# robustrobotics/flame_ros

Hardware: AMD Instinct MI355X
Metric: primal-dual iterations/sec on a 50000-vertex / 149966-edge Delaunay graph (higher is better)
Workload: dtype f32; 1 GPU; synthetic 50k-vertex Delaunay graph, 500 PD iterations per frame, one frame per GPU; V=50000, E=149966, parallelism=replicas1, num_tiles=256, tile_depth=4, tile_threads=1024, hipgraph=True, resident_solves_repeated=0

## Files before the change

flame_ros_amd/csrc/flame_hip.cpp:

```cpp
#include "../../include/flame_hip.h"

#include <hip/hip_runtime.h>
#include <roctracer/roctx.h>

#include <atomic>
#include <chrono>
#include <climits>
#include <cmath>
#include <cstdio>
#include <cstdlib>
#include <cstring>
#include <new>
#include <string>
#include <unordered_map>
#include <mutex>
#include <vector>

#include "delaunay_dev.h"
#include "kernels.h"
#include "plan.h"
#include "plan_dev.h"
#include "sync.h"

using namespace flamehip;
// ... 210 lines not shown
  PlanOptions opt;
  int num_cus = 0;
  int use_graph = 1;
  Plan plan;
  SyncOut sync;
  bool synced = false;
  int path = 0;

  hipStream_t stream = nullptr;
  hipStream_t stream_in = nullptr;
  DelaunayScratch dt;
  hipEvent_t ev0 = nullptr, ev1 = nullptr, ev_in = nullptr;
  hipEvent_t ev_state = nullptr;
  bool state_pending = false;
  float state_scale = 1.0f;
  bool timed = false;
  int last_launches = 0;

  float4* A[2] = {nullptr, nullptr};
  float4* B[2] = {nullptr, nullptr};
  float4* q[2] = {nullptr, nullptr};
  int cur = 0;
  int2* eij = nullptr;
  float4* ew = nullptr;
  int32_t* grow = nullptr;
  int32_t* ginc = nullptr;
  float2* pos = nullptr;
  TileDesc* tiles = nullptr;
  int32_t* t_vmap = nullptr;
  int32_t* t_emap = nullptr;
  uint2* t_eij = nullptr;
  float4* t_ew = nullptr;
  uint32_t* t_srow = nullptr;
  int32_t* tris = nullptr;
  int32_t* trow = nullptr;
  int32_t* tinc = nullptr;
  float4* tri_normals = nullptr;
  float4* vtx_normals = nullptr;
  uint8_t* tri_valid = nullptr;
  int64_t map_pixels = 0;
  uint32_t* map_owner = nullptr;
  float* map_idm = nullptr;
  float* map_dm = nullptr;
  float* map_cloud = nullptr;
  uint32_t* map_cov = nullptr;
  char* fr_dev = nullptr;
  uint32_t* dbg_key = nullptr;
  uint8_t* dbg_bgr = nullptr;
  float* dbg_feat = nullptr;
  uint64_t state_serial = 1, raster_serial = 0;
  int raster_filtered = -1;
  flame_hip_tri_params raster_tp;
  float raster_kinv[9];
  float* filter_tmp = nullptr;
  float4* mesh_pts = nullptr;
  int32_t* v_i2o_dev = nullptr;
  int32_t* v_o2i_dev = nullptr;
  int32_t* e_i2o_dev = nullptr;
  int32_t* e_o2i_dev = nullptr;
  float* dl_v = nullptr;
  float* dl_q = nullptr;
  float* dl_n = nullptr;
  int plan_device = 1;
  int plan_reuse = 1;
  int plan_mini = 1;
  bool plan_mini_used = false;
// ... 53 lines not shown
  int2* in_edges = nullptr;
  float* in_alpha = nullptr;
  float* in_beta = nullptr;
  float* in_z = nullptr;
  float* in_wgt = nullptr;
  float* in_x0 = nullptr;
  int32_t* in_tris = nullptr;
  float* in_mu = nullptr;
  float* in_var = nullptr;
  float* in_pred = nullptr;
  bool sync_on_device = false;
  bool beta_is_alpha = false;
  int32_t* dflags = nullptr;
  bool host_perms = true;
  double* partials = nullptr;
  uint8_t* cost_mask = nullptr;
  int32_t n_send_v = 0, n_send_e = 0, n_recv_v = 0, n_recv_e = 0;
  int32_t* halo_send_v = nullptr;
  int32_t* halo_send_e = nullptr;
  int32_t* halo_recv_v = nullptr;
  int32_t* halo_recv_e = nullptr;
  int profile = 0;
  unsigned long long* prof = nullptr;

  std::vector<GraphExecEntry> execs;
  CapMap caps;
  int solves_since_upload = 0;
  PinnedArena pin;
  PinnedArena pin_in;
  char* in_stage = nullptr;
  PinnedArena pout;
  char* harena = nullptr;
  bool lanes_applied = false;
  bool poll_valid = false;
  bool poll_sorted = false;

  void drop_execs() {
    for (auto& e : execs) (void)hipGraphExecDestroy(e.exec);
    execs.clear();
  }

  void free_device() {
    if (device < 0) return;
    (void)hipSetDevice(device);
    drop_execs();
    for (auto& kv : caps) {
      void** pp = reinterpret_cast<void**>(kv.first);
      if (*pp) (void)hipFree(*pp);
      *pp = nullptr;
    }
    caps.clear();
    for (int b = 0; b < 2; ++b) {
      float4** pp[3] = {&xp.hA[b], &xp.hB[b], &xp.hq[b]};
      for (int k = 0; k < 3; ++k) {
        if (*pp[k]) uncached_pool().give(device, *pp[k], xp_cap[3 * b + k]);
        *pp[k] = nullptr; xp_cap[3 * b + k] = 0;
      }
    }
    xp.prof = nullptr;
    xp.poll_v = nullptr; xp.poll_e = nullptr; xp.poll_ne = nullptr;
    xp.need_v = nullptr; xp.need_e = nullptr; xp.need_valid = false;
    pin.release();
    pin_in.release();
    pout.release();
    map_pixels = 0;
    n_send_v = n_send_e = n_recv_v = n_recv_e = 0;
// ... 178 lines not shown
  } else if (k == "host_threads") {
    if (value < 0) return FLAME_HIP_ERR_ARG;
    g->opt.host_threads = value;
  } else if (k == "tile_single_max") {
    if (value < 0 || value > 2048) return FLAME_HIP_ERR_ARG;
    g->opt.single_max = value;
  } else if (k == "debug_sub_cap") {
    g->opt.debug_sub_cap = value;
  } else if (k == "d_sign") {
    if (value != 1 && value != -1) return FLAME_HIP_ERR_ARG;
    g->opt.d_sign = value;
  } else if (k == "plan_device") {
    g->plan_device = value != 0;
  } else if (k == "plan_reuse") {
    g->plan_reuse = value != 0;
  } else if (k == "plan_mini") {
    g->plan_mini = value != 0;
  } else if (k == "stream_depth") {
    if (value < 0 || value > kMaxDepth) return FLAME_HIP_ERR_ARG;
    g->stream_depth = value;
  } else if (k == "persist") {
    g->persist = value != 0;
  } else if (k == "persist_prof") {
    if (value < 0) return FLAME_HIP_ERR_ARG;
    g->persist_prof_want = value;
  } else if (k == "one_xcd") {
    g->one_xcd_opt = value != 0;
  } else if (k == "poll_delay") {
    if (value < -1 || value > 255) return FLAME_HIP_ERR_ARG;
    g->poll_delay_opt = value;
  } else if (k == "persist_timeout_us") {
    if (value < 0) return FLAME_HIP_ERR_ARG;
    g->persist_timeout_opt = value;
  } else if (k == "need_marks") {
    g->need_marks = value != 0;
  } else if (k == "plan_timing") {
    if (value < 0 || value > 5) return FLAME_HIP_ERR_ARG;
    g->opt.timing = value;
  } else if (k == "profile") {
    g->profile = value != 0;
  } else if (k == "lds_bytes") {
    if (value < 1024) return FLAME_HIP_ERR_ARG;
    g->opt.lds_bytes = value;
  } else {
    return FLAME_HIP_ERR_ARG;
  }
  return 0;
}

int flame_hip_get_info(const flame_hip_graph* g, const char* key, int64_t* value) {
  if (!g || !key || !value) return FLAME_HIP_ERR_ARG;
  const std::string k(key);
  const Plan& P = g->plan;
  if (k == "V") *value = g->V;
  else if (k == "E") *value = g->E;
  else if (k == "T") *value = g->T;
  else if (k == "path") *value = g->path;
  else if (k == "num_tiles") *value = (int64_t)P.tiles.size();
  else if (k == "tile_threads") *value = P.tile_threads;
  else if (k == "tile_ept") *value = P.tile_ept;
  else if (k == "tile_vpt") *value = P.tile_vpt;
  else if (k == "tile_depth") *value = P.tile_depth;
  else if (k == "tile_lds_bytes") *value = P.tile_lds_bytes;
  else if (k == "tile_slot12") *value = P.tile_slot12 ? 1 : 0;
  else if (k == "tile_fat") *value = P.tile_fat ? 1 : 0;
  else if (k == "stall_hook_build") *value = tile_stall_hook_build() ? 1 : 0;
// ... 347 lines not shown

int flame_hip_graph_upload(flame_hip_graph* g, const float* pos, const int32_t* edges,
                           const float* alpha, const float* beta, const float* z,
                           const float* wgt, const float* x0, const int32_t* tris) {
  RoctxRange roctx_("flame_hip_graph_upload");
  if (!g) return FLAME_HIP_ERR_ARG;
  const int32_t V = g->V, E = g->E;
  if (edges != g->sync.edges.data()) g->synced = false;
  g->sync_on_device = false;
  g->beta_is_alpha = false;
  if ((V > 0 && (!pos || !z || !wgt)) || (E > 0 && (!edges || !alpha || !beta)))
    return FLAME_HIP_ERR_ARG;
  g->uploaded = false;
  const GraphOptScope opt_scope(g, V);
  int rc;
  auto device_plan = [&]() -> int {
    int r = upload_device_plan(g, pos, edges, alpha, beta, z, wgt, x0, tris);
    if (r <= 0) {
      (void)hipStreamSynchronize(g->stream);
      (void)hipStreamSynchronize(g->stream_in);
    }
    return r;
  };
  if (g->device >= 0) {
    HIPCHK(hipSetDevice(g->device));
    HIPCHK(wait_last_solve(g));
    HIPCHK(hipStreamSynchronize(g->stream));
    persist_discard(g);
    HIPCHK(hipStreamSynchronize(g->stream_in));
    HIPCHK(g->planner.wait_maps());
    g->drop_execs();
    g->solves_since_upload = 0;
    g->lanes_applied = false;
    rc = device_plan();
    if (rc < 0) return rc;
  } else {
    rc = 0;
  }
  bool dev_plan = rc == 1;
  if (!dev_plan) {
    if (!all_finite(pos, 2 * (size_t)V) || !all_finite(z, V) || !all_finite(wgt, V) ||
        !all_finite(alpha, E) || !all_finite(beta, E) || (x0 && !all_finite(x0, V)))
      return FLAME_HIP_ERR_NAN;
    g->plan.on_device = false;
    g->host_perms = true;
    const bool auto_single = g->device >= 0 && g->plan_device && g->opt.tile_own <= 0 && g->opt.batch_voff.empty() &&
                             plan_sizing(g->opt, V, E).single;
    g->opt.single_only = auto_single;
    rc = build_plan(g->opt, V, E, g->T, pos, edges, alpha, beta, tris, &g->plan);
    g->opt.single_only = false;
    if (rc == kPlanSingleNoFit) {
      g->single_cap = std::min(g->single_cap, std::max(V - 1, 0));
      g->opt.single_max = std::min(g->opt.single_max, g->single_cap);
      rc = device_plan();
      if (rc < 0) return rc;
      dev_plan = rc == 1;
      if (!dev_plan) {
        g->plan.on_device = false;
        g->host_perms = true;
        rc = build_plan(g->opt, V, E, g->T, pos, edges, alpha, beta, tris, &g->plan);
      }
    }
    if (!dev_plan && rc != 0) return rc;
  }
  const Plan& P = g->plan;
  if (!dev_plan) {
// ... 185 lines not shown
        if (!(sc > 0.0f)) sc = 1.0f;
      }
      auto al = [](size_t v) { return (v + 63) & ~(size_t)63; };
      const size_t o_tris = 0, o_pos = al(sizeof(int32_t) * 3 * (size_t)T), o_mu = o_pos + al(sizeof(float2) * (size_t)V);
      const size_t o_var = o_mu + al(sizeof(float) * (size_t)V), o_pred = o_var + al(sizeof(float) * (size_t)V);
      const size_t in_total = o_pred + (prediction ? al(sizeof(float) * (size_t)V) : 0);
      if ((rc = dev_alloc(g->caps, &g->in_stage, in_total))) return rc;
      HIPCHK(g->pin_in.reserve(in_total));
      if (!tris_dev) std::memcpy(g->pin_in.base + o_tris, tris, sizeof(int32_t) * 3 * (size_t)T);
      std::memcpy(g->pin_in.base + o_pos, pos, sizeof(float2) * (size_t)V);
      std::memcpy(g->pin_in.base + o_mu, idepth_mu, sizeof(float) * (size_t)V);
      std::memcpy(g->pin_in.base + o_var, idepth_var, sizeof(float) * (size_t)V);
      if (prediction) std::memcpy(g->pin_in.base + o_pred, prediction, sizeof(float) * (size_t)V);
      const char* src = g->pin_in.base;
      lap("H2D all");
      DevPlanner::MiniSync ms;
      ms.tris = tris_dev ? tris_dev : reinterpret_cast<const int32_t*>(src + o_tris);
      ms.pos = reinterpret_cast<const float2*>(src + o_pos);
      ms.mu = reinterpret_cast<const float*>(src + o_mu);
      ms.var = reinterpret_cast<const float*>(src + o_var);
      ms.pred = (use_pred) ? reinterpret_cast<const float*>(src + o_pred) : nullptr;
      ms.scale = sc;
      ms.adaptive = sp->adaptive_data_weights; ms.init_pred = sp->init_with_prediction;
      ms.z = g->in_z; ms.wgt = g->in_wgt; ms.x0 = g->in_x0; ms.edges = g->in_edges; ms.alpha = g->in_alpha;
      ms.dflags = g->dflags;
      g->planner.offer_mini(ms);
      const int32_t V0 = g->V, E0 = g->E, T0 = g->T;
      g->V = V; g->E = expected_E; g->T = T;
      g->uploaded = false;
      g->n_send_v = g->n_send_e = g->n_recv_v = g->n_recv_e = 0;
      g->drop_execs();
      g->solves_since_upload = 0;
      g->lanes_applied = false;
      g->beta_is_alpha = true;
      g->spec_edges = true;
      rc = upload_device_plan(g, nullptr, nullptr, nullptr, nullptr, nullptr, nullptr, nullptr, nullptr, true, true);
      g->spec_edges = false;
      g->planner.withdraw_mini();
      if (g->planner.mini_used() && rc == 1) {
        g->plan_mini_used = true;
        g->euler_backoff = 0;
        g->euler_off = (int32_t)((int64_t)g->E - V - T);
        if ((rc = finish_upload(g))) return rc;
        g->synced = true;
        g->sync_on_device = true;
        g->sync.scale = sc;
        if (scale) *scale = sc;
        return 0;
      }
      if (rc < 0) return rc;
      (void)hipStreamSynchronize(s);
      if (rc == 2 && g->planner.mini_used()) {
        g->euler_backoff = std::min(16, std::max(1, 2 * g->euler_backoff));
        g->euler_skip = g->euler_backoff;
        expected_E = -1;
      }
      g->V = V0; g->E = E0; g->T = T0;
      HIPCHK(hipMemsetAsync(g->dflags, 0, 8 * sizeof(int32_t), s));
    }
    if (tris_dev) {
      HIPCHK(hipMemcpyAsync(g->in_tris, tris_dev, sizeof(int32_t) * 3 * (size_t)T, hipMemcpyDeviceToDevice, s));
    } else {
      HIPCHK(stage(g->in_tris, tris, sizeof(int32_t) * 3 * (size_t)T));
      HIPCHK(staged_for());
    }
    lap("H2D triangles");
    HIPCHK(g->planner.edges_from_tris(s, V, T, g->in_tris, g->in_pos, g->in_edges, g->in_alpha, &E, &index_error, g->dflags,
                                      [&]() {
                                        stage_err = stage(g->in_mu, idepth_mu, sizeof(float) * (size_t)V);
                                        if (stage_err == hipSuccess) stage_err = stage(g->in_var, idepth_var, sizeof(float) * (size_t)V);
                                        if (stage_err == hipSuccess && prediction)
                                          stage_err = stage(g->in_pred, prediction, sizeof(float) * (size_t)V);
                                        if (stage_err == hipSuccess) stage_err = staged_for();
                                        vrc = validate();
                                        if (vrc == 0 && sp->rescale_data) {
                                          double acc = 0.0;
                                          for (int32_t v = 0; v < V; ++v) acc += (double)idepth_mu[v];
                                          sc = (float)(acc / (double)V);
                                          if (!(sc > 0.0f)) sc = 1.0f;
                                        }
                                      }, expected_E,
                                      [&]() {
                                        hipError_t e = stage(g->in_pos, pos, sizeof(float2) * (size_t)V);
                                        return e != hipSuccess ? e : staged_for();
                                      }));
    HIPCHK(stage_err);
    lap("edges_from_tris");
    if (vrc || index_error) g->uploaded = false;
    if (vrc) return vrc;
    if (index_error) return FLAME_HIP_ERR_ARG;
    HIPCHK(g->planner.sync_data(s, V, g->in_mu, g->in_var, use_pred ? g->in_pred : nullptr, sc, sp->adaptive_data_weights,
                                sp->init_with_prediction, g->in_z, g->in_wgt, g->in_x0, g->dflags));
    g->V = V; g->E = E; g->T = T;
    g->uploaded = false;
    g->n_send_v = g->n_send_e = g->n_recv_v = g->n_recv_e = 0;
    g->drop_execs();
    g->solves_since_upload = 0;
    g->lanes_applied = false;
    g->beta_is_alpha = true;
    g->spec_edges = expected_E >= 0;
    rc = upload_device_plan(g, nullptr, nullptr, nullptr, nullptr, nullptr, nullptr, nullptr, nullptr, true, true);
    g->spec_edges = false;
    if (rc == 2) {
      E = g->true_edges;
      g->euler_backoff = std::min(16, std::max(1, 2 * g->euler_backoff));
      g->euler_skip = g->euler_backoff;
      if (E < 0 || E > 3 * (int64_t)T) return FLAME_HIP_ERR_ARG;
      g->E = E;
      rc = upload_device_plan(g, nullptr, nullptr, nullptr, nullptr, nullptr, nullptr, nullptr, nullptr, true, true);
    } else if (expected_E >= 0) {
      g->euler_backoff = 0;
    }
    if (rc == 1 || rc == 0) g->euler_off = (int32_t)((int64_t)g->E - V - T);
    if (rc <= 0) (void)hipStreamSynchronize(s);
    if (rc < 0) return rc;
    if (rc == 1) {
      if ((rc = finish_upload(g))) return rc;
      g->synced = true;
      g->sync_on_device = true;
      g->sync.scale = sc;
      if (scale) *scale = sc;
      return 0;
    }
  }
  if ((rc = validate())) return rc;
  if (tris_dev && !(tris = g->dt.host_list())) return FLAME_HIP_ERR_HIP;
  rc = graph_sync_host(*sp, V, T, pos, idepth_mu, idepth_var, tris, prediction, &g->sync);
  if (rc) return rc;
  const int32_t E = (int32_t)(g->sync.edges.size() / 2);
  if ((rc = flame_hip_graph_resize(g, V, E, T))) return rc;
  const SyncOut& S = g->sync;
// ... 248 lines not shown
    return 1;
  }
  g->queued.clear(); g->qsnap_valid = false;
  const bool can = g->persist_used && unchecked <= 1 && g->state_serial == g->solve_serial + (uint64_t)own_marks && g->last_iters > 0;
  g->persist_used = false;
  if (!can) {
    g->uploaded = false;
    return FLAME_HIP_ERR_STATE;
  }
  hipStream_t s = g->last_stream ? g->last_stream : g->stream;
  int cur_out = 0, launches = 0;
  HIPCHK(hipEventRecord(g->ev0, s));
  g->persist_skip_once = true;
  int rc = enqueue_iterations(g, g->last_sp, g->last_iters, s, g->last_src, &cur_out, &launches);
  g->persist_skip_once = false;
  if (rc) return rc;
  g->cur = cur_out;
  g->state_serial++;
  g->last_launches = launches;
  HIPCHK(hipEventRecord(g->ev1, s));
  ++g->persist_recovered;
  return 1;
}

static int enqueue_iterations(flame_hip_graph* g, const SolveParams& sp, int32_t num_iters,
                              hipStream_t s, int cur, int* cur_out, int* launches) {
  const Plan& P = g->plan;
  *launches = 0;
  g->persist_used = false;
  if (g->path == FLAME_HIP_PATH_TILE) {
    TileArgs a;
    a.tiles = g->tiles; a.t_vmap = g->t_vmap; a.t_emap = g->t_emap; a.t_eij = g->t_eij;
    a.t_ew = g->t_ew; a.t_srow = g->t_srow; a.p = sp; a.ntiles = (int32_t)P.tiles.size();
    a.prof = g->prof;
    a.slot12 = P.tile_slot12 ? 1 : 0;
    a.fat = P.tile_fat ? 1 : 0;
    if (persist_applies(g, num_iters) && persist_lease_take(g, s, P.tile_fat && P.tile_depth <= 2)) {
      PersistBufs& x = g->xp;
      int rc;
      if (!g->persist_err) {
        HIPCHK(hipHostMalloc(reinterpret_cast<void**>(&g->persist_err), 64, hipHostMallocDefault));
        *g->persist_err = 0;
      }
      if (!x.prof || g->persist_prof_set != g->persist_prof_want) {
        if ((rc = dev_alloc(g->caps, &x.prof, 16))) return rc;
        int32_t w[16] = {0, 0, 0, 0, 0, 0, 0, 0, 0, 0, 0, 0, 0, 0, 0, 0};
        int want = g->persist_prof_want;
        if (want > 0) { w[0] = 1; w[1] = want - 1; }
        HIPCHK(memcpy_sync(s, x.prof, w, sizeof(w), hipMemcpyHostToDevice));
        g->persist_prof_set = g->persist_prof_want;
      }
      const int rounds = (num_iters + P.tile_depth - 1) / P.tile_depth;
      bool rezero = g->persist_base > (1 << 23);
      if (rezero) g->persist_base = 0;
      const bool want_sorted = g->solves_since_upload > 0;
      if (!g->poll_valid || (want_sorted && !g->poll_sorted)) {
        size_t nv_loc = 0, ne_loc = 0;
        for (const TileDesc& D : P.tiles) { nv_loc += (size_t)D.n_ext; ne_loc += (size_t)D.e_loc; }
        if ((rc = dev_alloc(g->caps, &x.poll_v, nv_loc + 1)) || (rc = dev_alloc(g->caps, &x.poll_e, ne_loc + 1)) ||
            (rc = dev_alloc(g->caps, &x.poll_ne, P.tiles.size())))
          return rc;
        x.need_valid = false;
        if (want_sorted && g->need_marks && P.tile_fat) {
          if ((rc = dev_alloc(g->caps, &x.need_v, std::max<size_t>((size_t)g->V, 1))) || (rc = dev_alloc(g->caps, &x.need_e, std::max<size_t>((size_t)g->E, 1))))
            return rc;
          HIPCHK(hipMemsetAsync(x.need_v, 0, sizeof(int32_t) * std::max<size_t>((size_t)g->V, 1), s));
          HIPCHK(hipMemsetAsync(x.need_e, 0, sizeof(int32_t) * std::max<size_t>((size_t)g->E, 1), s));
          x.need_valid = true;
        }
        HIPCHK(launch_poll_lists(s, (int32_t)P.tiles.size(), g->tiles, g->t_vmap, g->t_emap, g->t_eij, x.poll_v, x.poll_e, x.poll_ne, want_sorted,
                                 x.need_valid ? x.need_v : nullptr, x.need_valid ? x.need_e : nullptr));
        g->poll_sorted = want_sorted;
        x.stage_bytes = 0;
        for (const TileDesc& D : P.tiles) x.stage_bytes = std::max(x.stage_bytes, persist_stage_bytes(D));
        g->poll_valid = true;
      }
      for (int b = 0; b < 2; ++b) {
        float4** pp[3] = {&x.hA[b], &x.hB[b], &x.hq[b]};
        const size_t nn[3] = {(size_t)g->V, (size_t)g->V, (size_t)std::max(g->E, 1)};
        for (int k = 0; k < 3; ++k) {
          bool fresh = false;
          if ((rc = dev_alloc_uncached(g->device, pp[k], &g->xp_cap[3 * b + k], nn[k], &fresh))) return rc;
          if (fresh || rezero) HIPCHK(hipMemsetAsync(*pp[k], 0, g->xp_cap[3 * b + k], s));
        }
      }
      PersistBufs xl = x;
      g->one_xcd_used = false;
      if (g->one_xcd_opt && P.tiles.size() <= (size_t)kOneXcdTiles && g->num_cus >= 256 && one_xcd_allowed(g->device)) {
        for (int b = 0; b < 2; ++b) {
          float4** pp[3] = {&g->cA[b], &g->cB[b], &g->cq[b]};
          const size_t nn[3] = {(size_t)g->V, (size_t)g->V, (size_t)std::max(g->E, 1)};
          for (int k = 0; k < 3; ++k) {
            if ((rc = dev_alloc(g->caps, pp[k], nn[k]))) return rc;
            const size_t cap_now = g->caps[(void*)pp[k]];
            if (g->c_zeroed[3 * b + k] != (void*)*pp[k] || g->c_zeroed_cap[3 * b + k] != cap_now || rezero) {
              HIPCHK(hipMemsetAsync(*pp[k], 0, cap_now, s));
              g->c_zeroed[3 * b + k] = (void*)*pp[k];
              g->c_zeroed_cap[3 * b + k] = cap_now;
            }
          }
          xl.hA[b] = g->cA[b]; xl.hB[b] = g->cB[b]; xl.hq[b] = g->cq[b];
        }
        xl.one_xcd = 1;
// ... 44 lines not shown
      HIPCHK(launch_primal(s, g->V, g->grow, g->ginc, g->ew, g->q[cur], g->A[cur], g->B[cur], sp));
      *launches += 2;
    }
  }
  *cur_out = cur;
  return 0;
}

int flame_hip_solve(flame_hip_graph* g, const flame_hip_params* p, int32_t num_iters,
                    void* stream) {
  RoctxRange roctx_("flame_hip_solve");
  int rc = require_device(g);
  if (rc) return rc;
  if (!p || num_iters < 0) return FLAME_HIP_ERR_ARG;
  if (!std::isfinite(p->data_factor) || !std::isfinite(p->step_x) || !std::isfinite(p->step_q) ||
      !std::isfinite(p->theta) || std::isnan(p->x_min) || std::isnan(p->x_max))
    return FLAME_HIP_ERR_NAN;
  HIPCHK(hipSetDevice(g->device));
  hipStream_t s = stream ? (hipStream_t)stream : g->stream;
  SolveParams sp;
  sp.lambda = p->data_factor; sp.tau = p->step_x; sp.sigma = p->step_q; sp.theta = p->theta;
  sp.x_min = p->x_min; sp.x_max = p->x_max;
  sp.tl = p->step_x * p->data_factor;
  HIPCHK(order_after_state(g, s));
  if (g->path == FLAME_HIP_PATH_TILE && g->opt.lane_order == 1 && !g->lanes_applied &&
      g->solves_since_upload > 0 && num_iters > 0 && g->V > 0) {
    int e_max = 0;
    for (const TileDesc& D : g->plan.tiles) e_max = std::max(e_max, D.e_loc);
    if (g->timed) HIPCHK(hipStreamWaitEvent(s, g->ev1, 0));
    HIPCHK(launch_assign_lanes(s, (int32_t)g->plan.tiles.size(), e_max, g->tiles, g->t_eij, g->t_ew, g->t_emap, g->plan.tile_slot12));
    g->lanes_applied = true;
    g->poll_valid = false;
  }
  if (g->persist_unchecked_n == 0) { g->queued.clear(); g->qsnap_valid = false; }
  if (g->queued.size() == 1 && !g->qsnap_valid && g->state_serial == g->queued_serial + 1 && num_iters > 0) {
    int rc2;
    if ((rc2 = dev_alloc(g->caps, &g->qsnapA, (size_t)g->V)) || (rc2 = dev_alloc(g->caps, &g->qsnapB, (size_t)g->V)) ||
        (rc2 = dev_alloc(g->caps, &g->qsnapq, (size_t)std::max(g->E, 1))))
      return rc2;
    const int src = g->queued_src;
    HIPCHK(hipMemcpyAsync(g->qsnapA, g->A[src], sizeof(float4) * (size_t)g->V, hipMemcpyDeviceToDevice, s));
    HIPCHK(hipMemcpyAsync(g->qsnapB, g->B[src], sizeof(float4) * (size_t)g->V, hipMemcpyDeviceToDevice, s));
    if (g->E > 0) HIPCHK(hipMemcpyAsync(g->qsnapq, g->q[src], sizeof(float4) * (size_t)g->E, hipMemcpyDeviceToDevice, s));
    g->qsnap_valid = true;
  }
  const int cur_before = g->cur;
  const uint64_t serial_before = g->state_serial;
  HIPCHK(hipEventRecord(g->ev0, s));
  g->last_sp = sp; g->last_iters = num_iters; g->last_stream = s;
  g->persist_used = false;
  int launches = 0, cur_out = g->cur;
  if (num_iters > 0 && g->V > 0) {
    if (g->use_graph && g->solves_since_upload > 0 && !persist_applies(g, num_iters)) {
      GraphExecEntry* hit = nullptr;
      for (auto& e : g->execs)
        if (e.iters == num_iters && e.cur == g->cur && std::memcmp(&e.p, &sp, sizeof(sp)) == 0) hit = &e;
      if (!hit) {
        hipGraph_t graph = nullptr;
        HIPCHK(hipStreamBeginCapture(s, hipStreamCaptureModeRelaxed));
        rc = enqueue_iterations(g, sp, num_iters, s, g->cur, &cur_out, &launches);
        hipError_t ee = hipStreamEndCapture(s, &graph);
        if (rc) { if (graph) (void)hipGraphDestroy(graph); return rc; }
        HIPCHK(ee);
        hipGraphExec_t exec = nullptr;
        ee = hipGraphInstantiate(&exec, graph, nullptr, nullptr, 0);
        (void)hipGraphDestroy(graph);
// ... 565 lines not shown
  if (g->E > 0) HIPCHK(hipMemcpyAsync(g->q[g->cur], g->snapq, sizeof(float4) * (size_t)g->E, hipMemcpyDeviceToDevice, s));
  g->state_serial++;
  g->uploaded = true;
  return 0;
}

int flame_hip_persist_take_error(flame_hip_graph* g, int32_t* gave_up) {
  int rc = require_device(g);
  if (rc) return rc;
  if (!gave_up) return FLAME_HIP_ERR_ARG;
  const bool force_fail = TEST_HOOK(persist_fail, 0) != 0;
  *gave_up = 0;
  const bool had = g->persist_unchecked;
  g->persist_unchecked = false;
  g->persist_unchecked_n = 0;
  g->queued.clear(); g->qsnap_valid = false;
  if (had && g->persist_err && (*g->persist_err != 0 || force_fail)) {
    persist_note_give_up(g);
    *g->persist_err = 0;
    persist_lease_drop(g, true);
    g->persist_used = false;
    *gave_up = 1;
  }
  return 0;
}

int64_t flame_hip_debug_plan_array(const flame_hip_graph* g, const char* name, void* buf,
                                   int64_t cap_bytes) {
  if (!g || !name || !g->uploaded) return FLAME_HIP_ERR_ARG;
  const Plan& P = g->plan;
  const std::string k(name);
  const void* src = nullptr;
  int64_t n = 0, esz = 4;
  if (P.on_device && k != "tiles" && k != "profile" && k.compare(0, 5, "sync_") != 0) {
    int64_t nv = 0, ne = 0, ns = 0;
    for (const TileDesc& D : P.tiles) { nv += D.n_ext; ne += D.e_loc; ns += D.n_upd; }
    const void* dev = nullptr;
    const int64_t V = g->V, E = g->E;
    if (k == "v_o2i") { dev = g->v_o2i_dev; n = V; }
    else if (k == "v_i2o") { dev = g->v_i2o_dev; n = V; }
    else if (k == "e_o2i") { dev = g->e_o2i_dev; n = E; }
    else if (k == "e_i2o") { dev = g->e_i2o_dev; n = E; }
    else if (k == "grow") { dev = g->grow; n = V + 1; }
    else if (k == "ginc") { dev = g->ginc; n = 2 * E; }
    else if (k == "eij") { dev = g->eij; n = E; esz = 8; }
    else if (k == "ew") { dev = g->ew; n = E; esz = 16; }
    else if (k == "tris") { dev = g->tris; n = 3 * (int64_t)P.T; }
    else if (k == "trow") { dev = g->trow; n = P.T > 0 ? V + 1 : 0; }
    else if (k == "tinc") { dev = g->tinc; n = 3 * (int64_t)P.T; }
    else if (k == "t_vmap") { dev = g->t_vmap; n = nv; }
    else if (k == "t_emap") { dev = g->t_emap; n = ne; }
    else if (k == "t_eij") { dev = g->t_eij; n = ne; esz = 8; }
    else if (k == "t_ew") { dev = g->t_ew; n = ne; esz = 16; }
    else if (k == "t_srow") { dev = g->t_srow; n = ns; }
    else return FLAME_HIP_ERR_ARG;
    if (buf && cap_bytes > 0 && n > 0) {
      if (hipSetDevice(g->device) != hipSuccess ||
          memcpy_sync(g->stream, buf, dev, (size_t)std::min<int64_t>(cap_bytes, n * esz), hipMemcpyDeviceToHost) != hipSuccess)
        return FLAME_HIP_ERR_HIP;
    }
    return n;
  }
  if (g->lanes_applied && g->device >= 0 && (k == "t_emap" || k == "t_eij" || k == "t_ew")) {
    const void* dev = k == "t_emap" ? (const void*)g->t_emap : k == "t_eij" ? (const void*)g->t_eij : (const void*)g->t_ew;
    n = (int64_t)P.t_emap.size();
    esz = k == "t_emap" ? 4 : k == "t_eij" ? 8 : 16;
// ... 50 lines not shown
```

flame_ros_amd/csrc/plan_dev.h:

```cpp
#pragma once
#include <hip/hip_runtime.h>

#include <cstdint>
#include <functional>
#include <vector>

#include "common.h"
#include "plan.h"

namespace flamehip {

int test_alloc_fill();

struct DevPlanArrays {
  int32_t* v_o2i = nullptr;
  int32_t* v_i2o = nullptr;
  int32_t* e_o2i = nullptr;
  int32_t* e_i2o = nullptr;
  int2* eij = nullptr;
  float4* ew = nullptr;
  int32_t* grow = nullptr;
  int32_t* ginc = nullptr;
  int32_t* tris = nullptr;
  int32_t* trow = nullptr;
// ... 110 lines not shown
  int32_t* gadj_ = nullptr;
  int32_t* ipos_ = nullptr;
  int32_t* seg_tab_ = nullptr;
  int32_t* estart_ = nullptr;
  int32_t* tile_ext_ = nullptr;
  int32_t* tile_meta_ = nullptr;
  int32_t* flags_ = nullptr;
  unsigned long long* scan_agg_[2] = {nullptr, nullptr};
  uint32_t* scan_flag_[2] = {nullptr, nullptr};
  uint32_t scan_epoch_[2] = {0, 0};
  long long* grid_sum_ = nullptr;
  int32_t* grid_cnt_ = nullptr;
  int32_t* grid_w_ = nullptr;
  float* grid_bounds_ = nullptr;
  float* gbbox_ = nullptr;
  char* hpin_ = nullptr;
  size_t hpin_bytes_ = 0;
  hipStream_t s2_ = nullptr;
  hipEvent_t ev_fork_ = nullptr, ev_join_ = nullptr, ev_grid_ = nullptr;
  bool grid_pending_ = false;
  bool grid_deferred_ = false;
  struct GridJob { hipStream_t stream = nullptr; int32_t V = 0; const float2* pos = nullptr; const int32_t* v_i2o = nullptr;
                   const TileDesc* tiles = nullptr; } grid_job_;
  MiniSync mini_{};
  bool mini_set_ = false, mini_used_ = false;
  int64_t capV2_ = 0;
  size_t tcub_bytes_ = 0;
  void* tcub_tmp_ = nullptr;
  int32_t* tcnt_ = nullptr;
};

hipError_t launch_assign_lanes(hipStream_t s, int32_t ntiles, int32_t e_max, const TileDesc* tiles, uint2* t_eij,
                               float4* t_ew, int32_t* t_emap, bool slot12 = false);

}
```

flame_ros_amd/csrc/plan_dev.hip:

```cpp
#include "plan_dev.h"

#include <rocprim/block/block_radix_sort.hpp>
#include <rocprim/device/device_radix_sort.hpp>
#include <rocprim/device/device_scan.hpp>
#include <rocprim/functional.hpp>

#include <algorithm>
#include <chrono>
#include <climits>
#include <cmath>
#include <cstdio>
#include <cstdlib>

namespace flamehip {
namespace {

constexpr int kSegCap = 1024;
constexpr int kIdBits = 22;
constexpr int kEdgeBits = 24;
constexpr int kCapExt = 2048;
constexpr int kCapEdge = 6144;
constexpr int kSortPad = 8192;
constexpr int kHash = 4096;
constexpr int kMetaWords = 32;
// ... 1098 lines not shown
    const uint32_t s1b = ss != 0xffffu ? ss : (uint32_t)(nslots + best);
    const uint32_t s2b = sd != 0xffffu ? sd : (uint32_t)(nslots + best);
    if (lane == best) { used = true; got = k; }
    if (lane == rgb * 16 + (li & 15) && T_rs == 0) T_rs = li + 1;
    if (lane == rgb * 16 + (lj & 15) && T_rt == 0) T_rt = lj + 1;
    if (S12) {
      const int g16 = best >> 4, g32 = best >> 5;
      if (lane == g16 * 16 + (int)(s1b & 15)) ++T_ws;
      if (lane == g16 * 16 + (int)(s2b & 15)) ++T_wd;
      if (lane == g32 * 32 + (int)(s1b & 31)) ++T_ws1;
      if (lane == g32 * 32 + (int)(s2b & 31)) ++T_wd1;
    } else {
      if (lane == wgb * 8 + (int)(s1b & 7)) ++T_ws;
      if (lane == wgb * 8 + (int)(s2b & 7)) ++T_wd;
    }
  }
  const uint32_t nx = (uint32_t)__shfl((int)rec.x, got, 64), ny = (uint32_t)__shfl((int)rec.y, got, 64);
  const float wx = __shfl(w.x, got, 64), wy = __shfl(w.y, got, 64), wz = __shfl(w.z, got, 64), ww = __shfl(w.w, got, 64);
  const int32_t nm = __shfl(mp, got, 64);
  if (lane < c) {
    t_eij[eoff + b0 + lane] = make_uint2(nx, ny);
    t_ew[eoff + b0 + lane] = make_float4(wx, wy, wz, ww);
    t_emap[eoff + b0 + lane] = nm;
  }
}

template <bool S12>
__global__ __launch_bounds__(256) void k_assign_lanes(const TileDesc* __restrict__ tiles, uint2* t_eij, float4* t_ew,
                                                      int32_t* t_emap) {
  const TileDesc D = tiles[blockIdx.x];
  const int b0 = (blockIdx.y * 4 + (threadIdx.x >> 6)) * 64;
  if (D.n_ext <= 0 || b0 >= D.e_loc) return;
  assign_lanes_block<S12>(threadIdx.x & 63, b0, D.e_loc, D.erec_off, D.nslots, t_eij, t_ew, t_emap);
}

struct TileShared {
  int fail, ecnt, n;
  int32_t ring_end[kMaxDepth + 1], level_end[kMaxDepth + 1];
  int32_t gw[kCapExt / 64], gbase[kCapExt / 64 + 1];
};

struct TileOut {
  const float4* ew; TileDesc* tiles; int32_t* t_vmap; int32_t* t_emap; uint2* t_eij; float4* t_ew; uint32_t* t_srow;
  int32_t* flags; int lane_order;
  long long* prof;
};
#define TILE_STAMP(O, n) do { if ((O).prof && blockIdx.x == 0 && threadIdx.x == 0) (O).prof[n] = (long long)__builtin_amdgcn_s_memtime(); } while (0)

constexpr int kBucketInts = 2 * kCapExt + 8;

__device__ __forceinline__ int tile_bucket(const int32_t* ring_end, int lv, int rv, int kind) {
  const int rs = rv == 0 ? 0 : ring_end[rv - 1];
  return 2 * rs + (kind ? ring_end[rv] - rs : 0) + (lv - rs);
}

template <int NTB>
struct TileEmit {
  int32_t es, e_own, n_upd, eoff;
  const TileOut* O;
};

template <int NTB, bool EMIT>
__device__ __forceinline__ int tile_walk(const TileGraph& G, const TileLds& L, TileShared& S, int32_t* cnt, int n_ext,
                                         const TileEmit<NTB>* E) {
  static_assert(kRowLanes == 4 && NTB % 4 == 0, "groups of four lanes");
  const int tid = threadIdx.x, sub = tid & 3, lane0 = (tid & 63) & ~3;
// ... 1559 lines not shown
hipError_t DevPlanner::update_grid(hipStream_t s, int32_t V, int ntiles, const DevPlanInputs& in,
                                   const DevPlanArrays& A) {
  if (s2_) {
    HIPRET(hipEventRecord(ev_fork_, s));
    HIPRET(hipStreamWaitEvent(s2_, ev_fork_, 0));
  }
  grid_job_.stream = s2_ ? s2_ : s;
  grid_job_.V = V; grid_job_.pos = in.pos; grid_job_.v_i2o = A.v_i2o; grid_job_.tiles = A.tiles;
  grid_deferred_ = true;
  map_tiles_ = ntiles; map_V_ = V;
  grid_tiles_ = ntiles;
  return hipSuccess;
}

hipError_t DevPlanner::flush_grid(hipEvent_t after) {
  if (!grid_deferred_) return hipSuccess;
  grid_deferred_ = false;
  const int n = Plan::kGrid * Plan::kGrid;
  hipStream_t g2 = grid_job_.stream;
  if (after && s2_ && g2 == s2_) HIPRET(hipStreamWaitEvent(g2, after, 0));
  const int32_t V = grid_job_.V;
  zero4(g2, reinterpret_cast<int32_t*>(grid_sum_), 2 * (int64_t)n, grid_cnt_, n, cell_pyr_, kPyrAtomicCells);
  hipLaunchKernelGGL(k_grid_accum, grid1(V), dim3(256), 0, g2, V, grid_job_.pos, grid_job_.v_i2o, tile_of_int_,
                     grid_job_.tiles, gbbox_, reinterpret_cast<unsigned long long*>(grid_sum_), grid_cnt_, cell_pyr_);
  hipLaunchKernelGGL(k_grid_final, dim3(1), dim3(1024), 0, g2, V, reinterpret_cast<unsigned long long*>(grid_sum_),
                     grid_cnt_, grid_w_, gbbox_, grid_bounds_, cell_pyr_);
  if (s2_) {
    HIPRET(hipEventRecord(ev_grid_, s2_));
    grid_pending_ = true;
  }
  return hipGetLastError();
}

hipError_t launch_assign_lanes(hipStream_t s, int32_t ntiles, int32_t e_max, const TileDesc* tiles, uint2* t_eij,
                               float4* t_ew, int32_t* t_emap, bool slot12) {
  if (ntiles <= 0 || e_max <= 0) return hipSuccess;
  const unsigned by = (unsigned)((e_max + 255) / 256);
  if (slot12) hipLaunchKernelGGL(k_assign_lanes<true>, dim3((unsigned)ntiles, by), dim3(256), 0, s, tiles, t_eij, t_ew, t_emap);
  else hipLaunchKernelGGL(k_assign_lanes<false>, dim3((unsigned)ntiles, by), dim3(256), 0, s, tiles, t_eij, t_ew, t_emap);
  return hipGetLastError();
}

}
```

flame_ros_amd/regularizer.py:

```python
import ctypes as C

import numpy as np

from . import lib as _l
from .lib import Params, SyncParams, TriParams, FlameHipError


def default_params(data_factor=0.15, step_x=1e-3, step_q=125.0, theta=0.25, x_min=0.0, x_max=10.0):
    return Params(data_factor, step_x, step_q, theta, x_min, x_max)


def default_tri_params(width=640, height=480):
    return TriParams(1, 1.57, 0.35, 0.1, 1, 0.333, 1, 0.01, width, height)


def default_sync_params(adaptive_data_weights=False, rescale_data=False, init_with_prediction=True,
                        idepth_var_max_graph=0.01, edge_weight_rule=0, alpha_gain=0.0, beta_gain=0.0):
    return SyncParams(int(adaptive_data_weights), int(rescale_data), int(init_with_prediction),
                      idepth_var_max_graph, int(edge_weight_rule), float(alpha_gain), float(beta_gain))


def feature_gate(idepth_var, var_max):
    var = _f32(idepth_var)
    keep = np.empty(len(var), np.uint8)
# ... 130 lines not shown
            raise ValueError("array shapes do not match V/E")
        x0 = None if x0 is None else _f32(x0)
        if tris is not None:
            tris = np.ascontiguousarray(tris, dtype=np.int32).reshape(-1, 3)
        T = 0 if tris is None else tris.shape[0]
        _l.check(self._lib.flame_hip_graph_resize(self._h, V, E, T), "flame_hip_graph_resize")
        self.V, self.E, self.T = V, E, T
        _l.check(self._lib.flame_hip_graph_upload(self._h, _ptr(pos), _ptr(edges), _ptr(alpha),
                                                  _ptr(beta), _ptr(z), _ptr(wgt), _ptr(x0),
                                                  _ptr(tris)), "flame_hip_graph_upload")

    def close(self):
        if getattr(self, "_h", None):
            self._lib.flame_hip_graph_destroy(self._h)
            self._h = None

    def __del__(self):
        try:
            self.close()
        except Exception:
            pass

    def __enter__(self):
        return self

    def __exit__(self, *a):
        self.close()

    def info(self, key):
        v = C.c_int64()
        _l.check(self._lib.flame_hip_get_info(self._h, key.encode(), C.byref(v)), "flame_hip_get_info")
        return v.value

    _PLAN_ELEM_BYTES = {"eij": 8, "t_eij": 8, "ew": 16, "t_ew": 16, "profile": 8, "tiles": C.sizeof(_l.TileDesc)}

    def plan_array(self, name, dtype):
        n = self._lib.flame_hip_debug_plan_array(self._h, name.encode(), None, 0)
        if n < 0:
            raise FlameHipError(int(n), "flame_hip_debug_plan_array")
        nbytes = int(n) * self._PLAN_ELEM_BYTES.get(name, 4)
        out = np.zeros(nbytes // np.dtype(dtype).itemsize, dtype=dtype)
        if n:
            self._lib.flame_hip_debug_plan_array(self._h, name.encode(), _ptr(out), out.nbytes)
        return out

    def set_state(self, x=None, w1=None, w2=None, xb=None, w1b=None, w2b=None, q=None):
        arrs = [None if a is None else _f32(a) for a in (x, w1, w2, xb, w1b, w2b, q)]
        _l.check(self._lib.flame_hip_set_state(self._h, *[_ptr(a) for a in arrs]), "flame_hip_set_state")

    def step(self, params, num_iters=1, stream=None, sync=True):
        _l.check(self._lib.flame_hip_solve(self._h, C.byref(params), int(num_iters), stream),
                 "flame_hip_solve")
        if sync:
            self.sync()

    solve = step

    def sync(self):
        _l.check(self._lib.flame_hip_sync(self._h), "flame_hip_sync")

    def last_solve_ms(self):
        ms, n = C.c_float(), C.c_int32()
        _l.check(self._lib.flame_hip_last_solve_ms(self._h, C.byref(ms), C.byref(n)),
                 "flame_hip_last_solve_ms")
        return ms.value, n.value

    def costs(self, params):
# ... 96 lines not shown
```

Before: 760,700 PD iterations/s.

## Permute tile edge records within 64-lane blocks to reduce LDS bank conflicts

Adds a one-time device kernel that, after the first solve, greedily swaps edge records inside each 64-edge wavefront block to minimise a modelled LDS bank-conflict cost for the gather reads and slot writes. The permuted edge arrays are kept in separate buffers and used by the tile solver and the poll-list builder, and cached graph execs are rebuilt. It is on by default for non-slot12 tile plans. The aim is fewer LDS conflicts in every PD iteration, paid for with extra device memory and a one-off placement pass whose cost model may not match the hardware.

```diff
diff --git a/flame_ros_amd/csrc/flame_hip.cpp b/flame_ros_amd/csrc/flame_hip.cpp
--- a/flame_ros_amd/csrc/flame_hip.cpp
+++ b/flame_ros_amd/csrc/flame_hip.cpp
@@ -266,6 +266,9 @@
   uint2* t_eij = nullptr;
   float4* t_ew = nullptr;
   uint32_t* t_srow = nullptr;
+  uint2* p_eij = nullptr;
+  float4* p_ew = nullptr;
+  int32_t* p_emap = nullptr;
   int32_t* tris = nullptr;
   int32_t* trow = nullptr;
   int32_t* tinc = nullptr;
@@ -385,6 +388,8 @@
   PinnedArena pout;
   char* harena = nullptr;
   bool lanes_applied = false;
+  bool slot_place = true;
+  bool placed = false;
   bool poll_valid = false;
   bool poll_sorted = false;
 
@@ -629,6 +634,9 @@
   } else if (k == "persist_timeout_us") {
     if (value < 0) return FLAME_HIP_ERR_ARG;
     g->persist_timeout_opt = value;
+  } else if (k == "slot_place") {
+    g->slot_place = value != 0;
+    if (!g->slot_place && g->placed) { g->placed = false; g->poll_valid = false; g->drop_execs(); }
   } else if (k == "need_marks") {
     g->need_marks = value != 0;
   } else if (k == "plan_timing") {
@@ -1042,6 +1050,7 @@
     g->drop_execs();
     g->solves_since_upload = 0;
     g->lanes_applied = false;
+    g->placed = false;
     rc = device_plan();
     if (rc < 0) return rc;
   } else {
@@ -1293,6 +1302,7 @@
       g->drop_execs();
       g->solves_since_upload = 0;
       g->lanes_applied = false;
+    g->placed = false;
       g->beta_is_alpha = true;
       g->spec_edges = true;
       rc = upload_device_plan(g, nullptr, nullptr, nullptr, nullptr, nullptr, nullptr, nullptr, nullptr, true, true);
@@ -1358,6 +1368,7 @@
     g->drop_execs();
     g->solves_since_upload = 0;
     g->lanes_applied = false;
+    g->placed = false;
     g->beta_is_alpha = true;
     g->spec_edges = expected_E >= 0;
     rc = upload_device_plan(g, nullptr, nullptr, nullptr, nullptr, nullptr, nullptr, nullptr, nullptr, true, true);
@@ -1672,6 +1683,7 @@
     TileArgs a;
     a.tiles = g->tiles; a.t_vmap = g->t_vmap; a.t_emap = g->t_emap; a.t_eij = g->t_eij;
     a.t_ew = g->t_ew; a.t_srow = g->t_srow; a.p = sp; a.ntiles = (int32_t)P.tiles.size();
+    if (g->placed) { a.t_eij = g->p_eij; a.t_ew = g->p_ew; a.t_emap = g->p_emap; }
     a.prof = g->prof;
     a.slot12 = P.tile_slot12 ? 1 : 0;
     a.fat = P.tile_fat ? 1 : 0;
@@ -1708,7 +1720,7 @@
           HIPCHK(hipMemsetAsync(x.need_e, 0, sizeof(int32_t) * std::max<size_t>((size_t)g->E, 1), s));
           x.need_valid = true;
         }
-        HIPCHK(launch_poll_lists(s, (int32_t)P.tiles.size(), g->tiles, g->t_vmap, g->t_emap, g->t_eij, x.poll_v, x.poll_e, x.poll_ne, want_sorted,
+        HIPCHK(launch_poll_lists(s, (int32_t)P.tiles.size(), g->tiles, g->t_vmap, a.t_emap, a.t_eij, x.poll_v, x.poll_e, x.poll_ne, want_sorted,
                                  x.need_valid ? x.need_v : nullptr, x.need_valid ? x.need_e : nullptr));
         g->poll_sorted = want_sorted;
         x.stage_bytes = 0;
@@ -1819,6 +1831,21 @@
     g->lanes_applied = true;
     g->poll_valid = false;
   }
+  if (g->path == FLAME_HIP_PATH_TILE && g->slot_place && !g->placed && !g->plan.tile_slot12 && g->solves_since_upload > 0 &&
+      num_iters > 0 && g->V > 0) {
+    int e_max = 0;
+    size_t ne = 0;
+    for (const TileDesc& D : g->plan.tiles) { e_max = std::max(e_max, D.e_loc); ne = std::max(ne, (size_t)D.erec_off + (size_t)D.e_loc); }
+    int rc2;
+    if ((rc2 = dev_alloc(g->caps, &g->p_eij, ne)) || (rc2 = dev_alloc(g->caps, &g->p_ew, ne)) || (rc2 = dev_alloc(g->caps, &g->p_emap, ne)))
+      return rc2;
+    if (g->timed) HIPCHK(hipStreamWaitEvent(s, g->ev1, 0));
+    HIPCHK(launch_place_lanes(s, (int32_t)g->plan.tiles.size(), e_max, g->tiles, g->t_eij, g->t_ew, g->t_emap, g->p_eij, g->p_ew,
+                              g->p_emap));
+    g->placed = true;
+    g->poll_valid = false;
+    g->drop_execs();
+  }
   if (g->persist_unchecked_n == 0) { g->queued.clear(); g->qsnap_valid = false; }
   if (g->queued.size() == 1 && !g->qsnap_valid && g->state_serial == g->queued_serial + 1 && num_iters > 0) {
     int rc2;
@@ -2450,6 +2477,18 @@
   const std::string k(name);
   const void* src = nullptr;
   int64_t n = 0, esz = 4;
+  if (k == "placed_t_eij" || k == "placed_t_emap" || k == "placed_t_ew") {
+    if (!g->placed || g->device < 0) return FLAME_HIP_ERR_STATE;
+    const void* dev = k == "placed_t_emap" ? (const void*)g->p_emap : k == "placed_t_eij" ? (const void*)g->p_eij : (const void*)g->p_ew;
+    for (const TileDesc& D : P.tiles) n = std::max<int64_t>(n, (int64_t)D.erec_off + D.e_loc);
+    esz = k == "placed_t_emap" ? 4 : k == "placed_t_eij" ? 8 : 16;
+    if (buf && cap_bytes > 0 && n > 0) {
+      if (hipSetDevice(g->device) != hipSuccess ||
+          memcpy_sync(g->stream, buf, dev, (size_t)std::min<int64_t>(cap_bytes, n * esz), hipMemcpyDeviceToHost) != hipSuccess)
+        return FLAME_HIP_ERR_HIP;
+    }
+    return n;
+  }
   if (P.on_device && k != "tiles" && k != "profile" && k.compare(0, 5, "sync_") != 0) {
     int64_t nv = 0, ne = 0, ns = 0;
     for (const TileDesc& D : P.tiles) { nv += D.n_ext; ne += D.e_loc; ns += D.n_upd; }
diff --git a/flame_ros_amd/csrc/plan_dev.h b/flame_ros_amd/csrc/plan_dev.h
--- a/flame_ros_amd/csrc/plan_dev.h
+++ b/flame_ros_amd/csrc/plan_dev.h
@@ -166,5 +166,7 @@
 
 hipError_t launch_assign_lanes(hipStream_t s, int32_t ntiles, int32_t e_max, const TileDesc* tiles, uint2* t_eij,
                                float4* t_ew, int32_t* t_emap, bool slot12 = false);
+hipError_t launch_place_lanes(hipStream_t s, int32_t ntiles, int32_t e_max, const TileDesc* tiles, const uint2* t_eij,
+                              const float4* t_ew, const int32_t* t_emap, uint2* p_eij, float4* p_ew, int32_t* p_emap);
 
 }
diff --git a/flame_ros_amd/csrc/plan_dev.hip b/flame_ros_amd/csrc/plan_dev.hip
--- a/flame_ros_amd/csrc/plan_dev.hip
+++ b/flame_ros_amd/csrc/plan_dev.hip
@@ -1154,6 +1154,100 @@
   const int b0 = (blockIdx.y * 4 + (threadIdx.x >> 6)) * 64;
   if (D.n_ext <= 0 || b0 >= D.e_loc) return;
   assign_lanes_block<S12>(threadIdx.x & 63, b0, D.e_loc, D.erec_off, D.nslots, t_eij, t_ew, t_emap);
+}
+
+__device__ __forceinline__ int rd_group(int p) {
+  const int h = p & 31;
+  return ((h < 4 || (h >= 12 && h < 16) || (h >= 20 && h < 28)) ? 0 : 1) + 2 * (p >> 5);
+}
+__device__ __forceinline__ int max_byte(unsigned long long c) {
+  int m = 0;
+#pragma unroll
+  for (int k = 0; k < 8; ++k) m = max(m, (int)((c >> (8 * k)) & 0xffu));
+  return m;
+}
+__device__ int block_conflicts(const uint32_t* rx, const uint32_t* ry, int c, int32_t nslots, int i, int j) {
+  unsigned long long gat[2][4][2] = {};
+  unsigned long long wr[2][8] = {};
+  for (int p = 0; p < c; ++p) {
+    const int sp = p == i ? j : (p == j ? i : p);
+    const uint32_t x = rx[sp], y = ry[sp];
+    const int g = rd_group(p);
+#pragma unroll
+    for (int side = 0; side < 2; ++side) {
+      const uint32_t v = side ? x >> 16 : x & 0xffffu;
+      bool dup = false;
+      for (int q = 0; q < p && !dup; ++q) {
+        const int sq = q == i ? j : (q == j ? i : q);
+        dup = rd_group(q) == g && (side ? rx[sq] >> 16 : rx[sq] & 0xffffu) == v;
+      }
+      if (!dup) gat[side][g][(v >> 3) & 1] += 1ull << (8 * (v & 7));
+      const uint32_t s = side ? y >> 16 : y & 0xffffu;
+      const uint32_t sl = s != 0xffffu ? s : (uint32_t)(nslots + p);
+      wr[side][p >> 3] += 1ull << (8 * (sl & 7));
+    }
+  }
+  int cost = 0;
+#pragma unroll
+  for (int side = 0; side < 2; ++side) {
+#pragma unroll
+    for (int g = 0; g < 4; ++g) {
+      const int m = max(max_byte(gat[side][g][0]), max_byte(gat[side][g][1]));
+      cost += m > 0 ? m - 1 : 0;
+    }
+#pragma unroll
+    for (int w = 0; w < 8; ++w) {
+      const int m = max_byte(wr[side][w]);
+      cost += m > 0 ? m - 1 : 0;
+    }
+  }
+  return cost;
+}
+
+constexpr int kPlaceSweeps = 2;
+__global__ __launch_bounds__(256) void k_place_lanes(const TileDesc* __restrict__ tiles, const uint2* __restrict__ t_eij,
+                                                     const float4* __restrict__ t_ew, const int32_t* __restrict__ t_emap,
+                                                     uint2* p_eij, float4* p_ew, int32_t* p_emap) {
+  __shared__ uint32_t s_x[4][64], s_y[4][64];
+  __shared__ int s_perm[4][64];
+  const TileDesc D = tiles[blockIdx.x];
+  const int wv = threadIdx.x >> 6, lane = threadIdx.x & 63;
+  const int b0 = (blockIdx.y * 4 + wv) * 64;
+  if (D.n_ext <= 0 || b0 >= D.e_loc) return;
+  const int c = min(64, D.e_loc - b0);
+  const int src_i = D.erec_off + b0 + min(lane, c - 1);
+  const uint2 rec = t_eij[src_i];
+  uint32_t* rx = s_x[wv];
+  uint32_t* ry = s_y[wv];
+  rx[lane] = rec.x; ry[lane] = rec.y; s_perm[wv][lane] = lane;
+  __builtin_amdgcn_fence(__ATOMIC_ACQ_REL, "workgroup"); __builtin_amdgcn_wave_barrier();
+  int cur = block_conflicts(rx, ry, c, D.nslots, 0, 0);
+  for (int sweep = 0; sweep < kPlaceSweeps && cur > 0; ++sweep) {
+    for (int i = 0; i < c; ++i) {
+      const int cost = (lane < c && lane != i) ? block_conflicts(rx, ry, c, D.nslots, i, lane) : INT32_MAX;
+      int best = cost, bl = lane;
+#pragma unroll
+      for (int off = 32; off > 0; off >>= 1) {
+        const int oc = __shfl_xor(best, off, 64), ol = __shfl_xor(bl, off, 64);
+        if (oc < best || (oc == best && ol < bl)) { best = oc; bl = ol; }
+      }
+      if (best < cur) {
+        if (lane == 0) {
+          const uint32_t tx = rx[i], ty = ry[i]; const int tp = s_perm[wv][i];
+          rx[i] = rx[bl]; ry[i] = ry[bl]; s_perm[wv][i] = s_perm[wv][bl];
+          rx[bl] = tx; ry[bl] = ty; s_perm[wv][bl] = tp;
+        }
+        cur = best;
+        __builtin_amdgcn_fence(__ATOMIC_ACQ_REL, "workgroup"); __builtin_amdgcn_wave_barrier();
+      }
+    }
+  }
+  if (lane < c) {
+    const int from = D.erec_off + b0 + s_perm[wv][lane];
+    p_eij[D.erec_off + b0 + lane] = t_eij[from];
+    p_ew[D.erec_off + b0 + lane] = t_ew[from];
+    p_emap[D.emap_off + b0 + lane] = t_emap[D.emap_off + b0 + s_perm[wv][lane]];
+  }
 }
 
 struct TileShared {
@@ -2779,6 +2873,14 @@
   return hipGetLastError();
 }
 
+hipError_t launch_place_lanes(hipStream_t s, int32_t ntiles, int32_t e_max, const TileDesc* tiles, const uint2* t_eij,
+                              const float4* t_ew, const int32_t* t_emap, uint2* p_eij, float4* p_ew, int32_t* p_emap) {
+  if (ntiles <= 0 || e_max <= 0) return hipSuccess;
+  const unsigned by = (unsigned)((e_max + 255) / 256);
+  hipLaunchKernelGGL(k_place_lanes, dim3((unsigned)ntiles, by), dim3(256), 0, s, tiles, t_eij, t_ew, t_emap, p_eij, p_ew, p_emap);
+  return hipGetLastError();
+}
+
 hipError_t launch_assign_lanes(hipStream_t s, int32_t ntiles, int32_t e_max, const TileDesc* tiles, uint2* t_eij,
                                float4* t_ew, int32_t* t_emap, bool slot12) {
   if (ntiles <= 0 || e_max <= 0) return hipSuccess;
diff --git a/flame_ros_amd/regularizer.py b/flame_ros_amd/regularizer.py
--- a/flame_ros_amd/regularizer.py
+++ b/flame_ros_amd/regularizer.py
@@ -186,7 +186,7 @@
         _l.check(self._lib.flame_hip_get_info(self._h, key.encode(), C.byref(v)), "flame_hip_get_info")
         return v.value
 
-    _PLAN_ELEM_BYTES = {"eij": 8, "t_eij": 8, "ew": 16, "t_ew": 16, "profile": 8, "tiles": C.sizeof(_l.TileDesc)}
+    _PLAN_ELEM_BYTES = {"eij": 8, "t_eij": 8, "ew": 16, "t_ew": 16, "placed_t_eij": 8, "placed_t_ew": 16, "profile": 8, "tiles": C.sizeof(_l.TileDesc)}
 
     def plan_array(self, name, dtype):
         n = self._lib.flame_hip_debug_plan_array(self._h, name.encode(), None, 0)
```

After: 777,400 PD iterations/s, median of 6. 2.2% higher.
